# mahdeslami11/jalil-saboorizadeh-Multi-speaker-Neural-Vocoder

Hardware: AMD Instinct MI355X
Metric: audio samples/sec gen (3-tier dim1024) + TBPTT steps/sec @1/2/4/8 GPU (higher is better)
Workload: dtype bf16

## Files before the change

include/samplernn_hip.h:

```cpp
#ifndef SAMPLERNN_HIP_H
#define SAMPLERNN_HIP_H
#include <stddef.h>
#include <stdint.h>

#ifdef __cplusplus
extern "C" {
#endif

#define SRNN_MAX_TIERS 6
#define SRNN_MAX_RNN 4

const char* srnn_last_error(void);
int srnn_abi_version(void);
const char* srnn_build_hash(void);

int srnn_uquantize_f32(const float* x, int64_t* out, int64_t n, int q_levels, void* stream);
int srnn_uquantize_f64(const double* x, int64_t* out, int64_t n, int q_levels, void* stream);
int srnn_udequantize(const int64_t* k, float* out, int64_t n, int q_levels, float scale,
                     int mode, void* stream);
int srnn_udequantize2d(const int64_t* k, int64_t ldk, float* out, int rows, int cols,
                       int q_levels, float scale, int mode, void* stream);

int srnn_gemm(int dtype, int out_dtype, int transA, int transB, int M, int N, int K,
              float alpha, const void* A, int64_t lda, int64_t strideA, const void* B,
// ... 84 lines not shown
int srnn_gemm_amax_taken(void);
int srnn_gemm_amax_blk_next(unsigned* amax, void* blk);
int srnn_gemm_csum_next(float* part);
int srnn_gemm_csum_taken(void);
int srnn_gemm_logsoftmax_next(void);
int srnn_gemm_logsoftmax_taken(void);
int srnn_mlp_dtab4(int dtype, const void* da, int64_t ldda, const int64_t* x, int64_t ldx,
                   int xoff, int B, int Tlen, void* dtab_out, int out_dtype, int D, int FS0, int Q,
                   void* work, size_t work_bytes, float* colsum, int* colsum_done,
                   const unsigned* amax_in, const void* blk, void* stream);
int srnn_dtab_packed_ok(void);
int srnn_blaslt_calls(void);
int srnn_blaslt_set_min(long long min_outputs, double min_flop);
int srnn_blaslt_set_tune(int n);
int srnn_logsoftmax_bwd(const float* dlogp, int64_t lddl, const float* logp, int64_t ldl,
                        int64_t rows, int Q, void* dz, int dz_dtype, int64_t ldd, void* stream);
int srnn_nll_fwd(const float* logp, int64_t ldl, const int64_t* target, int64_t ldt, int Tlen,
                 int64_t rows, float* loss_row, void* stream);
int srnn_nll_bwd(const int64_t* target, int64_t ldt, int Tlen, int64_t rows, int Q,
                 float* dlogp, int64_t ldd, float gscale, const float* gmul, void* stream);
int srnn_nll_logsoftmax_bwd(const int64_t* target, int64_t ldt, int Tlen, int64_t rows, int Q,
                            const float* logp, int64_t ldl, float gscale, const float* gmul,
                            void* dz, int dz_dtype, int64_t ldd, void* stream);
int srnn_logsoftmax_nll(const float* z, int64_t ldz, const int64_t* target, int64_t ldt,
                        int Tlen, int64_t rows, int Q, float* loss_row, float* logp,
                        int64_t ldl, void* dz, int dz_dtype, int64_t ldd, float gscale,
                        void* stream);

int srnn_uquantize_f64_host(const double* x, int64_t* out, int64_t n, int q_levels);
int srnn_uquantize_f32_host(const float* x, int64_t* out, int64_t n, int q_levels);
int srnn_udequantize_host(const int64_t* k, float* out, int64_t n, int q_levels);

int srnn_weight_norm_fwd(const float* g, const float* v, float* w, float* norm, int O,
                         int64_t R, void* stream);
int srnn_weight_norm_bwd(const float* g, const float* v, const float* dw, float* dg, float* dv,
                         int O, int64_t R, int accumulate, void* stream);
int srnn_weight_norm_scale(const float* g, const float* v, float* scale, int O, int64_t R,
                           void* stream);
int srnn_convt_fold(const float* v, const float* scale, void* dst, int dst_dtype, int Cin,
                    int Cout, int k, void* stream);
int srnn_convt_wn_bwd(const float* g, const float* v, const float* dwt, float* dg, float* dv,
                      int Cin, int Cout, int k, void* stream);

int srnn_permute3(const float* src, void* dst, int dst_dtype, int d0, int d1, int d2, int p0,
                  int p1, int p2, int accumulate, void* stream);
int srnn_copy2d(int src_dtype, int dst_dtype, int rows, int cols, const void* src, int64_t lds,
                void* dst, int64_t ldd, void* stream);
int srnn_gather_rows(const float* table, int64_t ldt, const int64_t* idx, int64_t n, int cols,
                     void* out, int out_dtype, int64_t ldo, void* stream);
int srnn_scatter_add_rows(float* table, int64_t ldt, const int64_t* idx, int64_t n, int cols,
                          const float* src, int64_t lds, void* stream);
int srnn_index_add_rows(float* table, int64_t ldt, int trows, const int64_t* idx, int64_t n,
                        int cols, const float* src, int64_t lds, void* stream);
int srnn_axpby(float* out, const float* a, const float* b, float alpha, float beta, int64_t n,
               void* stream);
int srnn_add_bcast_rows(float* x, const float* v, int B, int F, int D, int64_t ldv, void* stream);
int srnn_segsum(const float* src, int64_t lds, int B, int F, int D, float* out, void* stream);
int srnn_colsum(int dtype, const void* src, int64_t lds, int64_t rows, int cols, float* out,
                float alpha, int accumulate, float* work, int64_t work_elems, void* stream);

int srnn_adam_clip(float* p, float* g, float* m, float* v, void* p_bf16, int64_t n,
                   float clip_lo, float clip_hi, double lr, double beta1, double beta2,
                   double eps, int64_t step, void* stream);
int srnn_adam_clip_multi(int ntensors, float* const* p, float* const* g, float* const* m,
                         float* const* v, void* const* p_bf16, const int64_t* n, float clip_lo,
                         float clip_hi, double lr, double beta1, double beta2, double eps,
                         int64_t step, void* stream);
int srnn_adam_clip_multi2(int ntensors, float* const* p, void* const* g, int gdtype, float gscale,
                          float* const* m, float* const* v, void* const* p_bf16, const int64_t* n,
                          float clip_lo, float clip_hi, double lr, double beta1, double beta2,
                          double eps, int64_t step, void* stream);
int srnn_adam_clip_multi3(int ntensors, float* const* p, void* const* g, int gdtype, float gscale,
                          float* const* m, float* const* v, void* const* p_bf16, const int64_t* n,
                          float clip_lo, float clip_hi, double lr, double beta1, double beta2,
                          double eps, int64_t step, const int64_t* dstep, void* stream);
int srnn_step_advance(int64_t* dstep, int n, void* stream);
int srnn_pack_grads(int ntensors, const float* const* src, const int64_t* n,
                    const int64_t* dst_off, void* flat, int dtype, void* stream);
int srnn_cast_multi(int ntensors, const float* const* src, void* const* dst, const int64_t* n,
                    void* stream);

typedef struct SrnnTier {
// ... 44 lines not shown
```

jalil-saboorizadeh-multi-speaker-neural-vocoder_amd/csrc/misc.hip:

```cpp
#include <type_traits>
#include <algorithm>

#include "samplernn_hip_internal.hpp"
#include "ulaw_tables.h"

__constant__ uint32_t c_ulaw_f32_steps[256];
__constant__ uint64_t c_ulaw_f64_thresh[256];
__constant__ uint32_t c_ulaw_lut[256];

static int g_tables_ready = 0;
static int ensure_tables() {
    if (g_tables_ready) return 0;
    SRNN_CHECK_HIP(hipMemcpyToSymbol(HIP_SYMBOL(c_ulaw_f32_steps), SRNN_ULAW_F32_STEPS_BITS,
                                     sizeof(SRNN_ULAW_F32_STEPS_BITS)));
    SRNN_CHECK_HIP(hipMemcpyToSymbol(HIP_SYMBOL(c_ulaw_f64_thresh), SRNN_ULAW_F64_THRESH_BITS,
                                     sizeof(SRNN_ULAW_F64_THRESH_BITS)));
    SRNN_CHECK_HIP(hipMemcpyToSymbol(HIP_SYMBOL(c_ulaw_lut), SRNN_ULAW_LUT_BITS,
                                     sizeof(SRNN_ULAW_LUT_BITS)));
    g_tables_ready = 1;
    return 0;
}
int srnn_init_tables() { return ensure_tables(); }

__device__ __forceinline__ int64_t uq_formula(double x, int q) {
// ... 707 lines not shown
    s = block_sum(s, sh);
    if (threadIdx.x == 0) dst[c] = accumulate ? dst[c] + alpha * s : alpha * s;
}

template <typename T>
static void colsum_pass(const T* src, int64_t lds, int64_t rows, int cols, int64_t rpb, int nrb,
                        float* dst, float alpha, int accumulate, bool final_, hipStream_t s) {
    const bool vec = (lds % 4 == 0) && ((uintptr_t)src % (4 * sizeof(T)) == 0);
    dim3 grid(cdiv(cols, 64), nrb);
    if (final_ && cols < 16 && nrb == 1) {
        hipLaunchKernelGGL((colsum_narrow_kernel<T>), dim3(cols), dim3(256), 0, s, src, lds, rows,
                           dst, alpha, accumulate);
        return;
    }
    if (final_) {
        if (vec) hipLaunchKernelGGL((colsum_kernel<T, true, true>), grid, dim3(256), 0, s, src, lds, rows, cols, rpb, dst, alpha, accumulate);
        else hipLaunchKernelGGL((colsum_kernel<T, false, true>), grid, dim3(256), 0, s, src, lds, rows, cols, rpb, dst, alpha, accumulate);
    } else {
        if (vec) hipLaunchKernelGGL((colsum_kernel<T, true, false>), grid, dim3(256), 0, s, src, lds, rows, cols, rpb, dst, alpha, accumulate);
        else hipLaunchKernelGGL((colsum_kernel<T, false, false>), grid, dim3(256), 0, s, src, lds, rows, cols, rpb, dst, alpha, accumulate);
    }
}

int srnn_colsum_impl(int dtype, const void* src, int64_t lds, int64_t rows, int cols, float* out,
                     float alpha, int accumulate, float* work, int64_t work_elems, hipStream_t s) {
    if (cols <= 0) return 0;
    const int cblk = cdiv(cols, 64);
    int64_t nrb = std::max<int64_t>(1, std::min<int64_t>(2048 / cblk, rows / 64));
    nrb = std::min<int64_t>(nrb, work_elems / cols);
    if (rows <= 256 && cblk >= 16) nrb = 1;
    if (rows <= 0 || nrb <= 1) {
        if (dtype == SRNN_F32)
            colsum_pass<float>((const float*)src, lds, rows, cols, std::max<int64_t>(rows, 1), 1,
                               out, alpha, accumulate, true, s);
        else
            colsum_pass<bf16>((const bf16*)src, lds, rows, cols, std::max<int64_t>(rows, 1), 1,
                              out, alpha, accumulate, true, s);
        SRNN_LAUNCH_CHECK();
        return 0;
    }
    const int64_t rpb = (rows + nrb - 1) / nrb;
    nrb = (rows + rpb - 1) / rpb;
    SRNN_REQUIRE(nrb * cols <= work_elems, "colsum: workspace too small");
    if (dtype == SRNN_F32)
        colsum_pass<float>((const float*)src, lds, rows, cols, rpb, (int)nrb, work, 1.f, 0, false, s);
    else
        colsum_pass<bf16>((const bf16*)src, lds, rows, cols, rpb, (int)nrb, work, 1.f, 0, false, s);
    SRNN_LAUNCH_CHECK();
    colsum_pass<float>(work, cols, nrb, cols, nrb, 1, out, alpha, accumulate, true, s);
    SRNN_LAUNCH_CHECK();
    return 0;
}

__global__ void segsum_kernel(const float* __restrict__ src, int64_t lds, int B, int F, int D,
                              float* __restrict__ out) {
    const int c = blockIdx.x * blockDim.x + threadIdx.x;
    const int b = blockIdx.y;
    if (c >= D) return;
    const float* p = src + (int64_t)b * F * lds + c;
    float s = 0.f;
    for (int f = 0; f < F; ++f) s += p[(int64_t)f * lds];
    out[(int64_t)b * D + c] = s;
}

extern "C" int srnn_segsum(const float* src, int64_t lds, int B, int F, int D, float* out,
                           void* stream) {
    if ((int64_t)B * D <= 0) return 0;
    hipLaunchKernelGGL(segsum_kernel, dim3(cdiv(D, 256), B), dim3(256), 0, (hipStream_t)stream,
                       src, lds, B, F, D, out);
    SRNN_LAUNCH_CHECK();
    return 0;
}

extern "C" int srnn_colsum(int dtype, const void* src, int64_t lds, int64_t rows, int cols,
                           float* out, float alpha, int accumulate, float* work,
                           int64_t work_elems, void* stream) {
    return srnn_colsum_impl(dtype, src, lds, rows, cols, out, alpha, accumulate, work, work_elems,
                            (hipStream_t)stream);
}

__global__ void adam_clip_kernel(float* __restrict__ p, float* __restrict__ g,
                                 float* __restrict__ m, float* __restrict__ v,
                                 bf16* __restrict__ p_lp, int64_t n, float lo, float hi, float w1,
                                 float b2, float omb2, float step_size, float bc2s, float eps) {
    int64_t i = (int64_t)blockIdx.x * blockDim.x + threadIdx.x;
    if (i >= n) return;
    float gi = fminf(fmaxf(g[i], lo), hi);
    g[i] = gi;
    float mi = m[i];
    mi = mi + w1 * (gi - mi);
    float vi = v[i] * b2;
    vi = vi + omb2 * gi * gi;
    float denom = sqrtf(vi) / bc2s + eps;
    float pi = p[i] + (-step_size) * mi / denom;
    m[i] = mi;
    v[i] = vi;
    p[i] = pi;
    if (p_lp) p_lp[i] = __float2bfloat16(pi);
}

#define ADAM_MT 64
// ... 288 lines not shown
```

jalil-saboorizadeh-multi-speaker-neural-vocoder_amd/csrc/mlp.hip:

```cpp
#include <algorithm>

#include "samplernn_hip_internal.hpp"
#include "sampler.hpp"

template <typename T, typename TU, int VPT>
__global__ __launch_bounds__(256) void mlp_l1_kernel(const T* __restrict__ tab,
                                                     const int64_t* __restrict__ x, int64_t ldx,
                                                     int xoff, const int* __restrict__ base,
                                                     int Tlen, const TU* __restrict__ upper,
                                                     int64_t ldu, T* __restrict__ out, int64_t ldo,
                                                     int D, int FS0, int Q) {
    const int64_t r = blockIdx.y;
    const int b = r / Tlen, t = r % Tlen;
    const int off = xoff + (base ? *base : 0);
    const int64_t* xr = x + (int64_t)b * ldx + off + t;
    const int o0 = (blockIdx.x * 256 + threadIdx.x) * VPT;
    if (o0 >= D) return;
    float acc[VPT];
    const TU* ur = upper + r * ldu + o0;
#pragma unroll
    for (int j = 0; j < VPT; ++j) acc[j] = to_f(ur[j]);
    constexpr int KMAX = 32;
    int qs[KMAX];
#pragma unroll
// ... 432 lines not shown
#pragma unroll
    for (int j = 0; j < 4; ++j) dz[r * ldd + lane + 64 * j] = from_f<TG>(g[j] - expf(p[j]) * s);
}

extern "C" int srnn_nll_logsoftmax_bwd(const int64_t* target, int64_t ldt, int Tlen,
                                       int64_t rows, int Q, const float* logp, int64_t ldl,
                                       float gscale, const float* gmul, void* dz, int dz_dtype,
                                       int64_t ldd, void* stream) {
    SRNN_REQUIRE(Q == 256, "nll_logsoftmax_bwd: q_levels must be 256");
    if (rows <= 0) return 0;
    dim3 grid(cdiv(rows, 4));
    if (dz_dtype == SRNN_BF16)
        hipLaunchKernelGGL((nll_logsoftmax_bwd_kernel<bf16>), grid, dim3(256), 0,
                           (hipStream_t)stream, target, ldt, Tlen, rows, logp, ldl, gscale, gmul,
                           (bf16*)dz, ldd);
    else
        hipLaunchKernelGGL((nll_logsoftmax_bwd_kernel<float>), grid, dim3(256), 0,
                           (hipStream_t)stream, target, ldt, Tlen, rows, logp, ldl, gscale, gmul,
                           (float*)dz, ldd);
    SRNN_LAUNCH_CHECK();
    return 0;
}

__global__ void nll_fwd_kernel(const float* __restrict__ lp, int64_t ldl,
                               const int64_t* __restrict__ target, int64_t ldt, int Tlen,
                               int64_t rows, float* __restrict__ loss_row) {
    const int64_t r = (int64_t)blockIdx.x * blockDim.x + threadIdx.x;
    if (r >= rows) return;
    const int64_t b = r / Tlen, t = r % Tlen;
    loss_row[r] = -lp[r * ldl + target[b * ldt + t]];
}

__global__ void nll_bwd_kernel(const int64_t* __restrict__ target, int64_t ldt, int Tlen,
                               int64_t rows, int Q, float* __restrict__ dl, int64_t ldd,
                               float gscale, const float* __restrict__ gmul) {
    const int64_t e = (int64_t)blockIdx.x * blockDim.x + threadIdx.x;
    if (e >= rows * Q) return;
    if (gmul) gscale *= *gmul;
    const int64_t r = e / Q;
    const int q = e % Q;
    const int64_t b = r / Tlen, t = r % Tlen;
    dl[r * ldd + q] = (q == target[b * ldt + t]) ? -gscale : 0.f;
}

extern "C" int srnn_nll_fwd(const float* logp, int64_t ldl, const int64_t* target, int64_t ldt,
                            int Tlen, int64_t rows, float* loss_row, void* stream) {
// ... 79 lines not shown
```

jalil-saboorizadeh-multi-speaker-neural-vocoder_amd/csrc/samplernn_hip_internal.hpp:

```cpp
#pragma once
#include "gemm_problem.hpp"

int srnn_relu_bits_impl(int dtype, const void* a, int64_t lda, int M, int N, unsigned short* bits,
                        int64_t ldb, hipStream_t s);

__host__ __device__ __forceinline__ int64_t srnn_bits_index(int64_t r, int g, int64_t M, int64_t ld) {
    return ld ? r * ld + g : (int64_t)g * M + r;
}

static inline int linear_fwd(int dt, int odt, int M, int N, int K, const void* x, int64_t ldx,
                             const void* W, int64_t ldw, const float* bias, void* y, int64_t ldy,
                             int relu, hipStream_t s, float beta = 0.f, const float* yin = nullptr,
                             int64_t ldyin = 0) {
    GemmProblem p;
    p.dtype = dt; p.out_dtype = odt; p.transB = 1;
    p.M = M; p.N = N; p.K = K; p.beta = beta;
    p.A = x; p.lda = ldx; p.B = W; p.ldb = ldw; p.C = y; p.ldc = ldy;
    p.Cin = yin; p.ldcin = ldyin; p.bias = bias; p.bias_mode = 1; p.relu = relu;
    return srnn_gemm_run(p, s);
}

int srnn_raise_lds(const void* kernel, int bytes);

static inline int env_flag(const char* name, int dflt) {
    const char* e = getenv(name);
    return (e && *e) ? atoi(e) : dflt;
}

int* srnn_sticky_flag();
int srnn_persist_spin_limit(int dflt);
int srnn_device_cus();
extern "C" int srnn_device_share(void);
int srnn_persist_fits_cus(int64_t blocks);
int srnn_persist_check(const void* kernel, int threads, size_t lds, int64_t blocks,
                       const char* what);

enum { SRNN_SCRATCH_SPLITK = 0, SRNN_SCRATCH_MASK = 1, SRNN_SCRATCH_NT = 2, SRNN_SCRATCH_BLASLT = 3,
       SRNN_SCRATCH_SLOTS = 4 };
void* srnn_scratch(int slot, size_t bytes);

float* srnn_splitk_scratch(size_t bytes);
int srnn_splitk_sum(const float* part, float* C, int64_t ldc, int M, int N, int ks, hipStream_t s);

int srnn_blaslt_enabled();
```

jalil-saboorizadeh-multi-speaker-neural-vocoder_amd/model.py:

```python
import ctypes
import os

import numpy as np
import torch
from torch.nn import init

import custom_ops
import nn
import utils
import samplernn_hip as H

verbose = False
_STATS = {'fused_colsum': 0, 'fused_lp': 0, 'csum_epi': 0, 'lsm_epi': 0, 'gru_xcd_fwd': 0, 'gru_xcd_bwd': 0, 'gru_seq': 0,
          'gru_cell_steps': 0, 'gru_cell_bwd_steps': 0}


def _default_dtype():
    v = os.environ.get('SRNN_COMPUTE_DTYPE', 'fp32').lower()
    return torch.bfloat16 if v in ('bf16', 'bfloat16') else torch.float32


class _GRUParams(torch.nn.Module):

    def __init__(self, input_size, hidden_size, num_layers):
        super().__init__()
        self.input_size, self.hidden_size, self.num_layers = input_size, hidden_size, num_layers
        for l in range(num_layers):
            isz = input_size if l == 0 else hidden_size
            self.register_parameter('weight_ih_l%d' % l,
                                    torch.nn.Parameter(torch.empty(3 * hidden_size, isz)))
            self.register_parameter('weight_hh_l%d' % l,
                                    torch.nn.Parameter(torch.empty(3 * hidden_size, hidden_size)))
            self.register_parameter('bias_ih_l%d' % l,
                                    torch.nn.Parameter(torch.empty(3 * hidden_size)))
            self.register_parameter('bias_hh_l%d' % l,
                                    torch.nn.Parameter(torch.empty(3 * hidden_size)))
        stdv = 1.0 / np.sqrt(hidden_size)
# ... 5 lines not shown

    def __init__(self, frame_sizes, n_rnn, dim, learn_h0, q_levels, ulaw, weight_norm, cond_dim,
                 spk_dim, qrnn=False):
        super().__init__()
        self.dim = dim
        self.q_levels = q_levels
        self.ulaw = ulaw
        self.cond_dim = cond_dim
        self.spk_dim = spk_dim
        self.frame_sizes = [int(f) for f in frame_sizes]
        self.n_rnn = n_rnn
        self.compute_dtype = _default_dtype()
        self.dequantize = utils.udequantize if ulaw else utils.linear_dequantize
        ns_frame_samples = list(map(int, np.cumprod(frame_sizes)))
        is_cond = [False] * len(frame_sizes)
        is_cond[-1] = True
        self.frame_level_rnns = torch.nn.ModuleList([
            FrameLevelRNN(frame_size, n_frame_samples, n_rnn, dim, learn_h0, c, cond_dim,
                          spk_dim, weight_norm, qrnn)
            for (frame_size, n_frame_samples, c) in zip(frame_sizes, ns_frame_samples, is_cond)
        ])
        self.sample_level_mlp = SampleLevelMLP(frame_sizes[0], dim, q_levels, weight_norm)
        self.frame_level_rnns[0].__dict__['_feeds_mlp'] = True
        for m in self.modules():
            if m is not self:
                m.__dict__['_root'] = self

    @property
    def lookback(self):
        return self.frame_level_rnns[-1].n_frame_samples


class FrameLevelRNN(torch.nn.Module):

    def __init__(self, frame_size, n_frame_samples, n_rnn, dim, learn_h0, is_cond, cond_dim,
                 spk_dim, w_norm, qrnn):
        super().__init__()
        self.frame_size = frame_size
        self.n_frame_samples = n_frame_samples
        self.dim = dim
        self.cond_dim = cond_dim
        self.spk_dim = spk_dim
        self.weight_norm = w_norm
        self.qrnn = qrnn
        self.n_rnn = n_rnn
        self.is_cond = is_cond
# ... 83 lines not shown
    if T is not None:
        return T
    root = mod.__dict__.get('_root')
    return root.compute_dtype if root is not None else torch.float32


class _Conv:

    def __init__(self, ts):
        if len(ts) == 2:
            self.weight_g, self.weight_v = ts
        else:
            self.weight = ts[0]


class TierSpec:

    def __init__(self, meta, ps):
        (self.dim, self.n_frame_samples, self.frame_size, self.n_rnn, is_cond, feeds, dt,
         wn_ie, wn_c, wn_s, wn_up) = [int(v) for v in meta[:11]]
        self.is_cond = bool(is_cond)
        self.T = torch.bfloat16 if dt else torch.float32
        self._feeds_mlp = bool(feeds)
        it = iter(ps)

        def take(wn):
            return _Conv([next(it) for _ in range(2 if wn else 1)])
        self.input_expand = take(wn_ie)
        next(it)
        if self.is_cond:
            self.cond_expand = take(wn_c)
            next(it)
            next(it)
            self.spk_expand = take(wn_s)
            next(it)
        for _ in range(4 * self.n_rnn):
            next(it)
        self.upsampling = _State()
        self.upsampling.conv_t = take(wn_up)


def tier_meta(mod):
    wn = lambda m: int(hasattr(m, 'weight_g'))
    return [mod.dim, mod.n_frame_samples, mod.frame_size, mod.n_rnn, int(mod.is_cond),
            int(bool(mod.__dict__.get('_feeds_mlp'))), H.dcode(_dt(mod)),
            wn(mod.input_expand), wn(mod.cond_expand) if mod.is_cond else 0,
            wn(mod.spk_expand) if mod.is_cond else 0, wn(mod.upsampling.conv_t)]


class MlpSpec:

    def __init__(self, meta, ps):
        self.q_levels, self.dim, self.frame_size, dt, wn = [int(v) for v in meta[:5]]
        self.T = torch.bfloat16 if dt else torch.float32
        it = iter(ps)

        def take():
            return _Conv([next(it) for _ in range(2 if wn else 1)])
        self.embedding = _Conv([next(it)])
        self.input = take()
        self.hidden = take()
        self.hidden.bias = next(it)
        self.output = take()
        self.output.bias = next(it)


def mlp_meta(mlp):
    return [mlp.q_levels, mlp.dim, mlp.frame_size, H.dcode(_dt(mlp)),
            int(hasattr(mlp.hidden, 'weight_g'))]

# ... 141 lines not shown
    r = sv[9:]
    Wih, Whh = r[:L], r[L:2 * L]
    xs, outs, outsT, gates = r[2 * L:3 * L], r[3 * L:4 * L], r[4 * L:5 * L], r[5 * L:6 * L]
    WhhF = r[6 * L:7 * L]
    hprevs = r[7 * L:8 * L]
    dev = dY.device
    st = H.stream
    M = B * Fr
    if dY.dtype == T:
        dY2 = dYT = dY.reshape(M, k * D).contiguous()
    else:
        dY2 = dY.reshape(M, k * D).float().contiguous()
        lpc = getattr(dY, '_srnn_lp', None)
        if lpc is not None and lpc[1] == dY._version and lpc[0].dtype == T and \
                lpc[0].numel() == dY2.numel() and dY2.data_ptr() == dY.data_ptr():
            dYT = lpc[0].reshape(M, k * D)
            _STATS['fused_lp'] += 1
        else:
            dYT = H.cast(dY2, T)
    dWupT = H.gemm(outsT[-1].reshape(M, D), dYT, transA=True)
    cs = getattr(dY, '_srnn_colsum', None)
    if cs is not None and cs[1] == dY._version and cs[2] == k and cs[0].numel() == k * D:
        db_up = cs[0]
        _STATS['fused_colsum'] += 1
    else:
        db_up = H.colsum(dY2, M, k * D)
    dX = H.gemm(dYT, W_up.reshape(k * D, D))
    g_up = nn.convt_grad_to_params(mod.upsampling.conv_t, dWupT)
    g_up_b = H.permute3(db_up.reshape(1, k, D), (0, 2, 1)).reshape(D, k)
    g_rnn = [None] * L
    dh_in = [None] * L
    for l in reversed(range(L)):
        dOut = dX.reshape(B, Fr, D)
        WhhT = H.permute3(WhhF[l].detach().reshape(1, 3 * D, D), (0, 2, 1), dtype=T)
        xbw = H.gru_xcd_bwd_work_bytes(T, B, D) if lp else 0
        seq = lp and (xbw > 0 or H.gru_seq_supported(T, B, D))
        ddir = [torch.empty((B, D), device=dev, dtype=torch.float32) for _ in range(2)]
        dGIT = bsum = None
        if xbw > 0:
            dGH = dGI = None
            dGHT = torch.empty((B, Fr, 3 * D), device=dev, dtype=T)
            dGIT = torch.empty((B, Fr, 3 * D), device=dev, dtype=T)
            bsum = torch.empty((B, 4 * D), device=dev, dtype=torch.float32)
        else:
            dGH = torch.empty((B, Fr, 3 * D), device=dev, dtype=torch.float32)
            dGHT = torch.empty((B, Fr, 3 * D), device=dev, dtype=T) if lp else dGH
            dGI = torch.empty((B, Fr, 3 * D), device=dev, dtype=torch.float32)
# ... 39 lines not shown
        hprevT = hprevs[l]
        if hprevT is None:
            hprevT = torch.empty((B, Fr, D), device=dev, dtype=T)
            H.lib().call('srnn_copy2d', H.F32, H.dcode(T), B, D, H.ptr(h_in[l]), D,
                         H.ptr(hprevT), Fr * D, st())
            if Fr > 1:
                H.lib().call('srnn_copy2d', H.dcode(T), H.dcode(T), B, (Fr - 1) * D,
                             H.ptr(outsT[l]), Fr * D, H.ptr(hprevT[:, 1:]), Fr * D, st())
        dW_hh = H.gemm(dGHT.reshape(M, 3 * D), hprevT.reshape(M, D), transA=True)
        if bsum is not None:
            bs = H.colsum(bsum, B, 4 * D)
            db_hh = bs[:3 * D]
            db_ih = torch.cat([bs[:2 * D], bs[3 * D:]])
            dGIT = dGIT.reshape(M, 3 * D)
        else:
            dGH2, dGI2 = dGH.reshape(M, 3 * D), dGI.reshape(M, 3 * D)
            db_hh = H.colsum(dGH2, M, 3 * D)
            dGIT = H.cast(dGI2, T)
            db_ih = H.colsum(dGI2, M, 3 * D)
        dW_ih = H.gemm(dGIT, xs[l], transA=True)
        dX = H.gemm(dGIT, Wih[l])
        g_rnn[l] = [dW_ih, dW_hh, db_ih, db_hh]
    dx0 = dX
    dx0T = H.cast(dx0, T)
    dW_ie = H.gemm(dx0T, prevT, transA=True)
    g_ie = nn.weight_grad_to_params(mod.input_expand, dW_ie.reshape(D, nfs, 1))
    g_ie_b = H.colsum(dx0, M, D)
    d_upper = dx0.reshape(B, Fr, D) if ctx.has_upper else None
    if d_upper is not None and dx0T is not dx0:
        d_upper._srnn_lp = (dx0T, d_upper._version)
    grads = g_ie + [g_ie_b]
    if mod.is_cond:
        C = condT.shape[1]
        S = spk_embT.shape[1]
        dW_c = H.gemm(dx0T, condT, transA=True)
        grads += nn.weight_grad_to_params(mod.cond_expand, dW_c.reshape(D, C, 1))
        grads += [g_ie_b.clone()]
        dspk = torch.empty((B, D), device=dev, dtype=torch.float32)
        H.lib().call('srnn_segsum', H.ptr(dx0), D, B, Fr, D, H.ptr(dspk), st())
        dspkT = H.cast(dspk, T)
        dW_s = H.gemm(dspkT, spk_embT, transA=True)
        db_s = H.colsum(dspk, B, D)
        demb = H.gemm(dspkT, W_s)
        dE = torch.zeros((S, S), device=dev, dtype=torch.float32)
        H.lib().call('srnn_index_add_rows', H.ptr(dE), S, S, H.ptr(spk_flat), B, S,
                     H.ptr(demb), S, st())
        grads += [dE]
        grads += nn.weight_grad_to_params(mod.spk_expand, dW_s.reshape(D, S, 1))
        grads += [db_s]
    for l in range(L):
        grads += g_rnn[l]
    grads += g_up + [g_up_b]
    dh0 = None
# ... 100 lines not shown
        logp = torch.empty((B * Tl, Q), device=dev, dtype=torch.float32)
        H.lib().call('srnn_logsoftmax_nll', H.ptr(z), Q, None, 0, Tl, B * Tl, Q, None,
                     H.ptr(logp), Q, None, H.F32, 0, 0.0, H.stream())
    ctx = _State()
    ctx.mlp = mlp
    ctx.T = T
    ctx.udt = upper.dtype
    ctx.dims = (B, Tl, D, Q, FS0)
    ctx.saved_tensors = (x, a1, a2, logp, Wp, ET, W_hid, W_out)
    ctx.bits = (m1, m2)
    ctx.W_t = W_t
    return logp.reshape(B, Tl, Q), ctx


def mlp_backward(ctx, dlogp, nll=None):
    mlp = ctx.mlp
    T = ctx.T
    B, Tl, D, Q, FS0 = ctx.dims
    x, a1, a2, logp, Wp, ET, W_hid, W_out = ctx.saved_tensors
    dev = logp.device
    st = H.stream
    M = B * Tl
    dz = torch.empty((M, Q), device=dev, dtype=T)
    if nll is not None:
        tg, Tt, gscale, gd = nll
        H.lib().call('srnn_nll_logsoftmax_bwd', H.ptr(tg), Tt, Tt, M, Q, H.ptr(logp), Q,
                     gscale, H.ptr(gd), H.ptr(dz), H.dcode(T), Q, st())
    else:
        dl = dlogp.reshape(M, Q).float().contiguous()
        H.lib().call('srnn_logsoftmax_bwd', H.ptr(dl), Q, H.ptr(logp), Q, M, Q, H.ptr(dz),
                     H.dcode(T), Q, st())
    dW_out = H.gemm(dz, a2, transA=True)
    db_out = H.colsum(dz, M, Q)
    m1, m2 = ctx.bits
    ctx.bits = None
    W_t = ctx.W_t
    ctx.W_t = None
    Wo, tB = (W_t[1], True) if W_t is not None else (W_out, False)
    csp = None
    if T == torch.bfloat16 and M % 256 == 0 and os.environ.get('SRNN_CSUM_EPI', '1') != '0':
        csp = torch.empty((M // 128, D), device=dev, dtype=torch.float32)
        H.lib().call('srnn_gemm_csum_next', H.ptr(csp))
    ev = H.roof_begin()
    if m2 is not None:
        da2 = H.gemm(dz, Wo, transB=tB, mask_bits=m2, out_dtype=T)
    else:
        da2 = H.gemm(dz, Wo, transB=tB, mask=a2, out_dtype=T)
    H.roof_end('mlp_da2_gemm', ev, 2.0 * M * D * Q)
    if csp is not None and not H.lib().dll.srnn_gemm_csum_taken():
        csp = None
    if csp is not None:
        _STATS['csum_epi'] += 1
    ev = H.roof_begin()
    dW_hid = H.gemm(da2, a1, transA=True)
    H.roof_end('mlp_dw_hid_gemm', ev, 2.0 * M * D * D)
    db_hid = H.colsum(csp, M // 128, D) if csp is not None else H.colsum(da2, M, D)
# ... 289 lines not shown
```

jalil-saboorizadeh-multi-speaker-neural-vocoder_amd/samplernn_hip.py:

```python
import ctypes
import sys
import time
import os
import weakref

import torch

HERE = os.path.dirname(os.path.abspath(__file__))
LIB_PATH = os.path.join(HERE, 'libsamplernn_hip.so')

F32, BF16 = 0, 1
MAX_TIERS, MAX_RNN = 6, 4

_P = ctypes.c_void_p
_I = ctypes.c_int
_L = ctypes.c_int64
_F = ctypes.c_float
_D = ctypes.c_double
_U64 = ctypes.c_uint64
_SZ = ctypes.c_size_t

_SIGS = {
    'srnn_uquantize_f32': [_P, _P, _L, _I, _P],
    'srnn_uquantize_f64': [_P, _P, _L, _I, _P],
# ... 54 lines not shown
    'srnn_gru_xcd_bwd': [_I, _I, _I, _I, _P, _L, _L, _P, _L, _L, _P, _L, _L, _P, _P, _P, _P, _P,
                         _L, _L, _P, _P, _SZ, _P],
    'srnn_gru_xcd_bwd2': [_I, _I, _I, _I, _P, _L, _L, _P, _L, _L, _P, _L, _L, _P, _P, _P, _P, _P,
                          _P, _P, _L, _L, _P, _P, _SZ, _P],
    'srnn_weight_norm_scale': [_P, _P, _P, _I, _L, _P],
    'srnn_convt_fold': [_P, _P, _P, _I, _I, _I, _I, _P],
    'srnn_convt_wn_bwd': [_P, _P, _P, _P, _P, _I, _I, _I, _P],
    'srnn_gen_workspace_size': [_P, _I, ctypes.POINTER(_SZ)],
    'srnn_generate': [_P, _I, _I, _P, _P, _P, _U64, _P, _P, _P, _SZ, _I, _P],
    'srnn_generate2': [_P, _I, _I, _P, _P, _P, _U64, _I, _P, _P, _P, _SZ, _I, _P],
    'srnn_generate3': [_P, _I, _I, _P, _P, _P, _U64, _I, _P, _P, _P, _SZ, _I, _P, _P, _P],
    'srnn_persistent_flag_to_f32': [_P, _P],
    'srnn_persistent_flag_or_f32': [_P, _P],
    'srnn_persistent_flag_snapshot': [_P, _P],
    'srnn_persistent_flag_to': [_P, _I, _P],
    'srnn_persistent_flag_or': [_P, _I, _P],
    'srnn_adam_clip_multi2': [_I, _P, _P, _I, _F, _P, _P, _P, _P, _F, _F, _D, _D, _D, _D, _L,
                              _P],
    'srnn_pack_grads': [_I, _P, _P, _P, _P, _I, _P],
    'srnn_adam_clip_multi3': [_I, _P, _P, _I, _F, _P, _P, _P, _P, _F, _F, _D, _D, _D, _D, _L,
                              _P, _P],
    'srnn_step_advance': [_P, _I, _P],
    'srnn_nll_logsoftmax_bwd': [_P, _L, _I, _L, _I, _P, _L, _F, _P, _P, _I, _L, _P],
}


class SrnnTier(ctypes.Structure):
    _fields_ = [('frame_size', _I), ('n_frame_samples', _I), ('in_dim', _I),
                ('w_in', _P), ('b_in', _P),
                ('w_ih', _P * MAX_RNN), ('b_ih', _P * MAX_RNN),
                ('w_hh', _P * MAX_RNN), ('b_hh', _P * MAX_RNN),
                ('w_up', _P), ('b_up', _P), ('h0', _P)]


class SrnnModel(ctypes.Structure):
    _fields_ = [('n_tiers', _I), ('n_rnn', _I), ('dim', _I), ('q_levels', _I),
                ('cond_dim', _I), ('dtype', _I), ('tier', SrnnTier * MAX_TIERS),
                ('tab', _P), ('w_hid', _P), ('b_hid', _P), ('w_out', _P), ('b_out', _P)]


class _Lib:
    def __init__(self, path):
        if not os.path.exists(path):
            raise ImportError('libsamplernn_hip.so not built (%s); run __graft_entry__.build()'
                              % path)
        self.dll = ctypes.CDLL(path)
# ... 336 lines not shown
    if out is None:
        out = torch.empty(cols, device=x.device, dtype=torch.float32)
    lds = cols if lds is None else lds
    nrb = max(1, min((rows + 63) // 64, 2048 // max(1, (cols + 63) // 64)))
    work = torch.empty(nrb * cols + 256, device=x.device, dtype=torch.float32)
    lib().call('srnn_colsum', dcode(x), ptr(x), lds, rows, cols, ptr(out), alpha, int(accumulate),
               ptr(work), work.numel(), stream())
    return out


def cast(x, dtype):
    need_cuda(x)
    if x.dtype == dtype:
        return x
    x = x.contiguous()
    out = torch.empty(x.shape, device=x.device, dtype=dtype)
    cols = x.shape[-1] if x.dim() > 0 else 1
    rows = x.numel() // max(cols, 1)
    lib().call('srnn_copy2d', dcode(x), dcode(out), rows, cols, ptr(x), cols, ptr(out), cols,
               stream())
    return out


_SHADOW = {}


def cast_param(p, dtype):
    if p.dtype == dtype:
        return p
    key = id(p)
    e = _SHADOW.get(key)
    if e is not None and e[0]() is p and e[1].dtype == dtype and e[2] == p.data_ptr() and \
            e[3] == p._version:
        return e[1]
    c = cast(p.detach(), dtype)
    if e is None or e[0]() is not p:
        weakref.finalize(p, _SHADOW.pop, key, None)
    _SHADOW[key] = (weakref.ref(p), c, p.data_ptr(), p._version)
    return c


def shadow_refreshed(p):
    e = _SHADOW.get(id(p))
    if e is not None and e[0]() is p and e[2] == p.data_ptr():
        _SHADOW[id(p)] = (e[0], e[1], p.data_ptr(), p._version)

# ... 67 lines not shown
```

Measured before the change: 40.71 million.

## Fuse column sums into NLL-logsoftmax backward and dx0 bf16 cast

Adds a kernel that computes the bf16 dz gradient of NLL+logsoftmax and accumulates its per-column bias gradient partials in the same pass. Also adds a fused cast+colsum kernel for the tier input gradient that emits the bf16 copy, the total column sum, and the k-strided sums the upper tier's upsampling bias gradient needs, so the upper tier can reuse them. The aim is to drop separate colsum passes over dz and dx0 in TBPTT backward. The dz column sum is now taken from the bf16-rounded values rather than a separate read.

```diff
diff --git a/include/samplernn_hip.h b/include/samplernn_hip.h
--- a/include/samplernn_hip.h
+++ b/include/samplernn_hip.h
@@ -130,6 +130,10 @@
 int srnn_nll_logsoftmax_bwd(const int64_t* target, int64_t ldt, int Tlen, int64_t rows, int Q,
                             const float* logp, int64_t ldl, float gscale, const float* gmul,
                             void* dz, int dz_dtype, int64_t ldd, void* stream);
+int srnn_nll_logsoftmax_bwd_csum(const int64_t* target, int64_t ldt, int Tlen, int64_t rows,
+                                 int Q, const float* logp, int64_t ldl, float gscale,
+                                 const float* gmul, void* dz, int dz_dtype, int64_t ldd,
+                                 float* part, int64_t part_rows, float* colsum, void* stream);
 int srnn_logsoftmax_nll(const float* z, int64_t ldz, const int64_t* target, int64_t ldt,
                         int Tlen, int64_t rows, int Q, float* loss_row, float* logp,
                         int64_t ldl, void* dz, int dz_dtype, int64_t ldd, float gscale,
@@ -166,6 +170,9 @@
 int srnn_segsum(const float* src, int64_t lds, int B, int F, int D, float* out, void* stream);
 int srnn_colsum(int dtype, const void* src, int64_t lds, int64_t rows, int cols, float* out,
                 float alpha, int accumulate, float* work, int64_t work_elems, void* stream);
+int srnn_cast_colsum(const float* src, int64_t lds, int64_t rows, int cols, int k, void* dst,
+                     int dst_dtype, int64_t ldd, float* sums, float* total, float* work,
+                     int64_t work_elems, void* stream);
 
 int srnn_adam_clip(float* p, float* g, float* m, float* v, void* p_bf16, int64_t n,
                    float clip_lo, float clip_hi, double lr, double beta1, double beta2,
diff --git a/jalil-saboorizadeh-multi-speaker-neural-vocoder_amd/csrc/misc.hip b/jalil-saboorizadeh-multi-speaker-neural-vocoder_amd/csrc/misc.hip
--- a/jalil-saboorizadeh-multi-speaker-neural-vocoder_amd/csrc/misc.hip
+++ b/jalil-saboorizadeh-multi-speaker-neural-vocoder_amd/csrc/misc.hip
@@ -753,13 +753,31 @@
     }
 }
 
-int srnn_colsum_impl(int dtype, const void* src, int64_t lds, int64_t rows, int cols, float* out,
-                     float alpha, int accumulate, float* work, int64_t work_elems, hipStream_t s) {
-    if (cols <= 0) return 0;
+int64_t srnn_colsum_plan(int64_t rows, int cols, int64_t work_elems, int64_t* rpb) {
     const int cblk = cdiv(cols, 64);
     int64_t nrb = std::max<int64_t>(1, std::min<int64_t>(2048 / cblk, rows / 64));
     nrb = std::min<int64_t>(nrb, work_elems / cols);
     if (rows <= 256 && cblk >= 16) nrb = 1;
+    if (rows <= 0 || nrb <= 1) {
+        *rpb = std::max<int64_t>(rows, 1);
+        return 1;
+    }
+    *rpb = (rows + nrb - 1) / nrb;
+    return (rows + *rpb - 1) / *rpb;
+}
+
+int srnn_colsum_final(const float* work, int64_t nrb, int cols, float* out, float alpha,
+                      int accumulate, hipStream_t s) {
+    colsum_pass<float>(work, cols, nrb, cols, nrb, 1, out, alpha, accumulate, true, s);
+    SRNN_LAUNCH_CHECK();
+    return 0;
+}
+
+int srnn_colsum_impl(int dtype, const void* src, int64_t lds, int64_t rows, int cols, float* out,
+                     float alpha, int accumulate, float* work, int64_t work_elems, hipStream_t s) {
+    if (cols <= 0) return 0;
+    int64_t rpb;
+    const int64_t nrb = srnn_colsum_plan(rows, cols, work_elems, &rpb);
     if (rows <= 0 || nrb <= 1) {
         if (dtype == SRNN_F32)
             colsum_pass<float>((const float*)src, lds, rows, cols, std::max<int64_t>(rows, 1), 1,
@@ -770,17 +788,13 @@
         SRNN_LAUNCH_CHECK();
         return 0;
     }
-    const int64_t rpb = (rows + nrb - 1) / nrb;
-    nrb = (rows + rpb - 1) / rpb;
     SRNN_REQUIRE(nrb * cols <= work_elems, "colsum: workspace too small");
     if (dtype == SRNN_F32)
         colsum_pass<float>((const float*)src, lds, rows, cols, rpb, (int)nrb, work, 1.f, 0, false, s);
     else
         colsum_pass<bf16>((const bf16*)src, lds, rows, cols, rpb, (int)nrb, work, 1.f, 0, false, s);
     SRNN_LAUNCH_CHECK();
-    colsum_pass<float>(work, cols, nrb, cols, nrb, 1, out, alpha, accumulate, true, s);
-    SRNN_LAUNCH_CHECK();
-    return 0;
+    return srnn_colsum_final(work, nrb, cols, out, alpha, accumulate, s);
 }
 
 __global__ void segsum_kernel(const float* __restrict__ src, int64_t lds, int B, int F, int D,
@@ -808,6 +822,132 @@
                            int64_t work_elems, void* stream) {
     return srnn_colsum_impl(dtype, src, lds, rows, cols, out, alpha, accumulate, work, work_elems,
                             (hipStream_t)stream);
+}
+
+__device__ __forceinline__ unsigned cc_pack2(float a, float b) {
+    const bf16 x = from_f<bf16>(a), y = from_f<bf16>(b);
+    return (unsigned)*reinterpret_cast<const unsigned short*>(&x) |
+           ((unsigned)*reinterpret_cast<const unsigned short*>(&y) << 16);
+}
+
+template <bool VEC>
+__global__ __launch_bounds__(256) void cast_colsum_kernel(const float* __restrict__ src,
+                                                          int64_t lds, bf16* __restrict__ dst,
+                                                          int64_t ldd, int64_t rows, int cols,
+                                                          int k, int64_t rpb,
+                                                          float* __restrict__ part) {
+    __shared__ float red[16][129];
+    const int tx = threadIdx.x & 15, ty = threadIdx.x >> 4;
+    const int c = blockIdx.x * 128 + tx * 8;
+    const int64_t r0 = (int64_t)blockIdx.y * rpb;
+    const int64_t r1 = min(rows, r0 + rpb);
+    float s[8];
+#pragma unroll
+    for (int e = 0; e < 8; ++e) s[e] = 0.f;
+    if (VEC && c + 7 < cols) {
+        int64_t r = r0 + ty;
+        for (; r + 16 < r1; r += 32) {
+            floatx4 v[2][2];
+#pragma unroll
+            for (int u = 0; u < 2; ++u) {
+                const floatx4* p = reinterpret_cast<const floatx4*>(src + (r + 16 * u) * lds + c);
+                v[u][0] = p[0]; v[u][1] = p[1];
+            }
+#pragma unroll
+            for (int u = 0; u < 2; ++u) {
+                uint4 o;
+                o.x = cc_pack2(v[u][0][0], v[u][0][1]); o.y = cc_pack2(v[u][0][2], v[u][0][3]);
+                o.z = cc_pack2(v[u][1][0], v[u][1][1]); o.w = cc_pack2(v[u][1][2], v[u][1][3]);
+                *reinterpret_cast<uint4*>(dst + (r + 16 * u) * ldd + c) = o;
+#pragma unroll
+                for (int e = 0; e < 4; ++e) { s[e] += v[u][0][e]; s[4 + e] += v[u][1][e]; }
+            }
+        }
+        for (; r < r1; r += 16) {
+            const floatx4* p = reinterpret_cast<const floatx4*>(src + r * lds + c);
+            const floatx4 v0 = p[0], v1 = p[1];
+            uint4 o;
+            o.x = cc_pack2(v0[0], v0[1]); o.y = cc_pack2(v0[2], v0[3]);
+            o.z = cc_pack2(v1[0], v1[1]); o.w = cc_pack2(v1[2], v1[3]);
+            *reinterpret_cast<uint4*>(dst + r * ldd + c) = o;
+#pragma unroll
+            for (int e = 0; e < 4; ++e) { s[e] += v0[e]; s[4 + e] += v1[e]; }
+        }
+    } else {
+        for (int64_t r = r0 + ty; r < r1; r += 16)
+#pragma unroll
+            for (int e = 0; e < 8; ++e)
+                if (c + e < cols) {
+                    const float v = src[r * lds + c + e];
+                    dst[r * ldd + c + e] = from_f<bf16>(v);
+                    s[e] += v;
+                }
+    }
+#pragma unroll
+    for (int e = 0; e < 8; ++e) red[ty][tx * 8 + e] = s[e];
+    __syncthreads();
+    for (int o = threadIdx.x; o < k * 128; o += 256) {
+        const int j = o >> 7, cc = o & 127;
+        float t = 0.f;
+        for (int i = j; i < 16; i += k) t += red[i][cc];
+        if (blockIdx.x * 128 + cc < cols)
+            part[((int64_t)blockIdx.y * k + j) * cols + blockIdx.x * 128 + cc] = t;
+    }
+}
+
+__global__ __launch_bounds__(256) void cc_final_kernel(const float* __restrict__ part, int nrb,
+                                                       int k, int cols, float* __restrict__ sums,
+                                                       float* __restrict__ total) {
+    __shared__ float red[16][17];
+    const int tx = threadIdx.x & 15, ty = threadIdx.x >> 4;
+    const int c = blockIdx.x * 16 + tx;
+    float tot = 0.f;
+    for (int j = 0; j < k; ++j) {
+        float s = 0.f;
+        if (c < cols)
+            for (int b = ty; b < nrb; b += 16) s += part[((int64_t)b * k + j) * cols + c];
+        red[ty][tx] = s;
+        __syncthreads();
+        if (ty == 0) {
+            float t = 0.f;
+#pragma unroll
+            for (int i = 0; i < 16; ++i) t += red[i][tx];
+            if (c < cols && sums) sums[(int64_t)j * cols + c] = t;
+            tot += t;
+        }
+        __syncthreads();
+    }
+    if (ty == 0 && c < cols) total[c] = tot;
+}
+
+extern "C" int srnn_cast_colsum(const float* src, int64_t lds, int64_t rows, int cols, int k,
+                                void* dst, int dst_dtype, int64_t ldd, float* sums,
+                                float* total, float* work, int64_t work_elems, void* stream) {
+    SRNN_REQUIRE(dst_dtype == SRNN_BF16, "cast_colsum: dst must be bf16");
+    SRNN_REQUIRE(k >= 1 && k <= 16 && 16 % k == 0, "cast_colsum: k must divide 16");
+    SRNN_REQUIRE(rows > 0 && cols > 0, "cast_colsum: empty input");
+    SRNN_REQUIRE(total != nullptr, "cast_colsum: total is required");
+    const int cblk = cdiv(cols, 128);
+    int64_t nrb = std::max<int64_t>(1, std::min<int64_t>(1024 / cblk, rows / 64));
+    int64_t rpb = (rows + nrb - 1) / nrb;
+    rpb = (rpb + 15) / 16 * 16;
+    nrb = (rows + rpb - 1) / rpb;
+    SRNN_REQUIRE(work && work_elems >= nrb * k * cols, "cast_colsum: workspace too small");
+    const bool vec = lds % 4 == 0 && ldd % 8 == 0 && (uintptr_t)src % 16 == 0 &&
+                     (uintptr_t)dst % 16 == 0;
+    hipStream_t s = (hipStream_t)stream;
+    dim3 grid(cblk, (unsigned)nrb);
+    if (vec)
+        hipLaunchKernelGGL((cast_colsum_kernel<true>), grid, dim3(256), 0, s, src, lds, (bf16*)dst,
+                           ldd, rows, cols, k, rpb, work);
+    else
+        hipLaunchKernelGGL((cast_colsum_kernel<false>), grid, dim3(256), 0, s, src, lds,
+                           (bf16*)dst, ldd, rows, cols, k, rpb, work);
+    SRNN_LAUNCH_CHECK();
+    hipLaunchKernelGGL(cc_final_kernel, dim3(cdiv(cols, 16)), dim3(256), 0, s, work, (int)nrb, k,
+                       cols, sums, total);
+    SRNN_LAUNCH_CHECK();
+    return 0;
 }
 
 __global__ void adam_clip_kernel(float* __restrict__ p, float* __restrict__ g,
diff --git a/jalil-saboorizadeh-multi-speaker-neural-vocoder_amd/csrc/mlp.hip b/jalil-saboorizadeh-multi-speaker-neural-vocoder_amd/csrc/mlp.hip
--- a/jalil-saboorizadeh-multi-speaker-neural-vocoder_amd/csrc/mlp.hip
+++ b/jalil-saboorizadeh-multi-speaker-neural-vocoder_amd/csrc/mlp.hip
@@ -478,6 +478,83 @@
     return 0;
 }
 
+__global__ __launch_bounds__(1024) void nll_logsoftmax_bwd_csum_kernel(
+    const int64_t* __restrict__ target, int64_t ldt, int Tlen, int64_t rows,
+    const float* __restrict__ lp, int64_t ldl, float gscale, const float* __restrict__ gmul,
+    bf16* __restrict__ dz, int64_t ldd, int64_t rpb, float* __restrict__ part) {
+    __shared__ float red[16][256];
+    const int wave = threadIdx.x >> 6, lane = threadIdx.x & 63;
+    if (gmul) gscale *= *gmul;
+    const int64_t r0 = (int64_t)blockIdx.x * rpb + wave;
+    const int64_t r1 = min(rows, (int64_t)(blockIdx.x + 1) * rpb);
+    float cs[4] = {0.f, 0.f, 0.f, 0.f};
+    int64_t b = r0 / Tlen;
+    int64_t t = r0 - b * Tlen;
+    for (int64_t rb = r0; rb < r1; rb += 64) {
+        int tq[4];
+        float p[4][4];
+#pragma unroll
+        for (int u = 0; u < 4; ++u) {
+            const int64_t r = rb + 16 * u;
+            if (r < r1) {
+                tq[u] = (int)target[b * ldt + t];
+#pragma unroll
+                for (int j = 0; j < 4; ++j) p[u][j] = lp[r * ldl + lane + 64 * j];
+                t += 16;
+                while (t >= Tlen) {
+                    t -= Tlen;
+                    ++b;
+                }
+            }
+        }
+#pragma unroll
+        for (int u = 0; u < 4; ++u) {
+            const int64_t r = rb + 16 * u;
+            if (r < r1) {
+                float g[4];
+#pragma unroll
+                for (int j = 0; j < 4; ++j) g[j] = (lane + 64 * j == tq[u]) ? -gscale : 0.f;
+                const float s = wave_sum(g[0] + g[1] + g[2] + g[3]);
+#pragma unroll
+                for (int j = 0; j < 4; ++j) {
+                    const bf16 v = from_f<bf16>(g[j] - expf(p[u][j]) * s);
+                    dz[r * ldd + lane + 64 * j] = v;
+                    cs[j] += to_f(v);
+                }
+            }
+        }
+    }
+#pragma unroll
+    for (int j = 0; j < 4; ++j) red[wave][lane + 64 * j] = cs[j];
+    __syncthreads();
+    if (threadIdx.x < 256) {
+        const int c = threadIdx.x;
+        float t = 0.f;
+#pragma unroll
+        for (int i = 0; i < 16; ++i) t += red[i][c];
+        part[(int64_t)blockIdx.x * 256 + c] = t;
+    }
+}
+
+extern "C" int srnn_nll_logsoftmax_bwd_csum(const int64_t* target, int64_t ldt, int Tlen,
+                                            int64_t rows, int Q, const float* logp, int64_t ldl,
+                                            float gscale, const float* gmul, void* dz,
+                                            int dz_dtype, int64_t ldd, float* part,
+                                            int64_t part_rows, float* colsum, void* stream) {
+    SRNN_REQUIRE(Q == 256, "nll_logsoftmax_bwd_csum: q_levels must be 256");
+    SRNN_REQUIRE(dz_dtype == SRNN_BF16, "nll_logsoftmax_bwd_csum: dz must be bf16");
+    SRNN_REQUIRE(colsum != nullptr, "nll_logsoftmax_bwd_csum: colsum is required");
+    if (rows <= 0) return 0;
+    int64_t rpb;
+    const int64_t nb = srnn_colsum_plan(rows, Q, INT64_MAX, &rpb);
+    SRNN_REQUIRE(part && part_rows >= nb, "nll_logsoftmax_bwd_csum: partials too small");
+    hipLaunchKernelGGL(nll_logsoftmax_bwd_csum_kernel, dim3((unsigned)nb), dim3(1024), 0,
+                       (hipStream_t)stream, target, ldt, Tlen, rows, logp, ldl, gscale, gmul,
+                       (bf16*)dz, ldd, rpb, part);
+    SRNN_LAUNCH_CHECK();
+    return srnn_colsum_final(part, nb, Q, colsum, 1.f, 0, (hipStream_t)stream);
+}
+
 __global__ void nll_fwd_kernel(const float* __restrict__ lp, int64_t ldl,
                                const int64_t* __restrict__ target, int64_t ldt, int Tlen,
                                int64_t rows, float* __restrict__ loss_row) {
diff --git a/jalil-saboorizadeh-multi-speaker-neural-vocoder_amd/csrc/samplernn_hip_internal.hpp b/jalil-saboorizadeh-multi-speaker-neural-vocoder_amd/csrc/samplernn_hip_internal.hpp
--- a/jalil-saboorizadeh-multi-speaker-neural-vocoder_amd/csrc/samplernn_hip_internal.hpp
+++ b/jalil-saboorizadeh-multi-speaker-neural-vocoder_amd/csrc/samplernn_hip_internal.hpp
@@ -42,4 +42,8 @@
 float* srnn_splitk_scratch(size_t bytes);
 int srnn_splitk_sum(const float* part, float* C, int64_t ldc, int M, int N, int ks, hipStream_t s);
 
+int64_t srnn_colsum_plan(int64_t rows, int cols, int64_t work_elems, int64_t* rpb);
+int srnn_colsum_final(const float* work, int64_t nrb, int cols, float* out, float alpha,
+                      int accumulate, hipStream_t s);
+
 int srnn_blaslt_enabled();
diff --git a/jalil-saboorizadeh-multi-speaker-neural-vocoder_amd/model.py b/jalil-saboorizadeh-multi-speaker-neural-vocoder_amd/model.py
--- a/jalil-saboorizadeh-multi-speaker-neural-vocoder_amd/model.py
+++ b/jalil-saboorizadeh-multi-speaker-neural-vocoder_amd/model.py
@@ -12,7 +12,8 @@
 
 verbose = False
 _STATS = {'fused_colsum': 0, 'fused_lp': 0, 'csum_epi': 0, 'lsm_epi': 0, 'gru_xcd_fwd': 0, 'gru_xcd_bwd': 0, 'gru_seq': 0,
-          'gru_cell_steps': 0, 'gru_cell_bwd_steps': 0}
+          'gru_cell_steps': 0, 'gru_cell_bwd_steps': 0, 'dz_csum': 0, 'dx0_fused': 0,
+          'tier_colsum': 0}
 
 
 def _default_dtype():
@@ -64,6 +65,8 @@
         ])
         self.sample_level_mlp = SampleLevelMLP(frame_sizes[0], dim, q_levels, weight_norm)
         self.frame_level_rnns[0].__dict__['_feeds_mlp'] = True
+        for lo, up in zip(self.frame_level_rnns[:-1], self.frame_level_rnns[1:]):
+            lo.__dict__['_upper_k'] = up.frame_size
         for m in self.modules():
             if m is not self:
                 m.__dict__['_root'] = self
@@ -193,6 +196,7 @@
         self.is_cond = bool(is_cond)
         self.T = torch.bfloat16 if dt else torch.float32
         self._feeds_mlp = bool(feeds)
+        self._upper_k = int(meta[11]) if len(meta) > 11 else 0
         it = iter(ps)
 
         def take(wn):
@@ -216,7 +220,8 @@
     return [mod.dim, mod.n_frame_samples, mod.frame_size, mod.n_rnn, int(mod.is_cond),
             int(bool(mod.__dict__.get('_feeds_mlp'))), H.dcode(_dt(mod)),
             wn(mod.input_expand), wn(mod.cond_expand) if mod.is_cond else 0,
-            wn(mod.spk_expand) if mod.is_cond else 0, wn(mod.upsampling.conv_t)]
+            wn(mod.spk_expand) if mod.is_cond else 0, wn(mod.upsampling.conv_t),
+            int(mod.__dict__.get('_upper_k') or 0)]
 
 
 class MlpSpec:
@@ -404,7 +409,7 @@
     cs = getattr(dY, '_srnn_colsum', None)
     if cs is not None and cs[1] == dY._version and cs[2] == k and cs[0].numel() == k * D:
         db_up = cs[0]
-        _STATS['fused_colsum'] += 1
+        _STATS[cs[3] if len(cs) > 3 else 'fused_colsum'] += 1
     else:
         db_up = H.colsum(dY2, M, k * D)
     dX = H.gemm(dYT, W_up.reshape(k * D, D))
@@ -490,13 +495,22 @@
         dX = H.gemm(dGIT, Wih[l])
         g_rnn[l] = [dW_ih, dW_hh, db_ih, db_hh]
     dx0 = dX
-    dx0T = H.cast(dx0, T)
+    k_up = int(getattr(mod, '_upper_k', 0) or 0) if ctx.has_upper else 1
+    cs_up = None
+    if T == torch.bfloat16 and dx0.dtype == torch.float32 and H.cast_colsum_ok(k_up) and \
+            M % k_up == 0 and os.environ.get('SRNN_DX0_FUSED', '1') != '0':
+        dx0T, cs_up, g_ie_b = H.cast_colsum(dx0, M, D, k_up)
+        _STATS['dx0_fused'] += 1
+    else:
+        dx0T = H.cast(dx0, T)
+        g_ie_b = H.colsum(dx0, M, D)
     dW_ie = H.gemm(dx0T, prevT, transA=True)
     g_ie = nn.weight_grad_to_params(mod.input_expand, dW_ie.reshape(D, nfs, 1))
-    g_ie_b = H.colsum(dx0, M, D)
     d_upper = dx0.reshape(B, Fr, D) if ctx.has_upper else None
     if d_upper is not None and dx0T is not dx0:
         d_upper._srnn_lp = (dx0T, d_upper._version)
+    if d_upper is not None and cs_up is not None:
+        d_upper._srnn_colsum = (cs_up.reshape(-1), d_upper._version, k_up, 'tier_colsum')
     grads = g_ie + [g_ie_b]
     if mod.is_cond:
         C = condT.shape[1]
@@ -643,16 +657,22 @@
     st = H.stream
     M = B * Tl
     dz = torch.empty((M, Q), device=dev, dtype=T)
+    db_out = None
     if nll is not None:
         tg, Tt, gscale, gd = nll
-        H.lib().call('srnn_nll_logsoftmax_bwd', H.ptr(tg), Tt, Tt, M, Q, H.ptr(logp), Q,
-                     gscale, H.ptr(gd), H.ptr(dz), H.dcode(T), Q, st())
+        if T == torch.bfloat16 and os.environ.get('SRNN_DZ_CSUM', '1') != '0':
+            db_out = H.nll_logsoftmax_bwd_csum(tg, Tt, M, Q, logp, gscale, gd, dz)
+            _STATS['dz_csum'] += 1
+        else:
+            H.lib().call('srnn_nll_logsoftmax_bwd', H.ptr(tg), Tt, Tt, M, Q, H.ptr(logp), Q,
+                         gscale, H.ptr(gd), H.ptr(dz), H.dcode(T), Q, st())
     else:
         dl = dlogp.reshape(M, Q).float().contiguous()
         H.lib().call('srnn_logsoftmax_bwd', H.ptr(dl), Q, H.ptr(logp), Q, M, Q, H.ptr(dz),
                      H.dcode(T), Q, st())
     dW_out = H.gemm(dz, a2, transA=True)
-    db_out = H.colsum(dz, M, Q)
+    if db_out is None:
+        db_out = H.colsum(dz, M, Q)
     m1, m2 = ctx.bits
     ctx.bits = None
     W_t = ctx.W_t
diff --git a/jalil-saboorizadeh-multi-speaker-neural-vocoder_amd/samplernn_hip.py b/jalil-saboorizadeh-multi-speaker-neural-vocoder_amd/samplernn_hip.py
--- a/jalil-saboorizadeh-multi-speaker-neural-vocoder_amd/samplernn_hip.py
+++ b/jalil-saboorizadeh-multi-speaker-neural-vocoder_amd/samplernn_hip.py
@@ -100,6 +100,9 @@
                               _P, _P],
     'srnn_step_advance': [_P, _I, _P],
     'srnn_nll_logsoftmax_bwd': [_P, _L, _I, _L, _I, _P, _L, _F, _P, _P, _I, _L, _P],
+    'srnn_nll_logsoftmax_bwd_csum': [_P, _L, _I, _L, _I, _P, _L, _F, _P, _P, _I, _L, _P, _L, _P,
+                                     _P],
+    'srnn_cast_colsum': [_P, _L, _L, _I, _I, _P, _I, _L, _P, _P, _P, _L, _P],
 }
 
 
@@ -482,6 +485,33 @@
     return out
 
 
+def nll_logsoftmax_bwd_csum(target, Tlen, rows, Q, logp, gscale, gmul, dz):
+    need_cuda(logp)
+    part = torch.empty((max(1, min(512, rows // 64)), Q), device=logp.device, dtype=torch.float32)
+    out = torch.empty(Q, device=logp.device, dtype=torch.float32)
+    lib().call('srnn_nll_logsoftmax_bwd_csum', ptr(target), Tlen, Tlen, rows, Q, ptr(logp), Q,
+               gscale, ptr(gmul), ptr(dz), BF16, Q, ptr(part), part.shape[0], ptr(out), stream())
+    return out
+
+
+def cast_colsum_ok(k):
+    return 1 <= k <= 16 and 16 % k == 0
+
+
+def cast_colsum(x, rows, cols, k=1):
+    need_cuda(x)
+    x = x.contiguous()
+    dev = x.device
+    out = torch.empty((rows, cols), device=dev, dtype=torch.bfloat16)
+    sums = torch.empty((k, cols), device=dev, dtype=torch.float32)
+    total = torch.empty(cols, device=dev, dtype=torch.float32)
+    nrb = max(1, min(1024 // ((cols + 127) // 128), rows // 64))
+    work = torch.empty(nrb * k * cols, device=dev, dtype=torch.float32)
+    lib().call('srnn_cast_colsum', ptr(x), cols, rows, cols, k, ptr(out), BF16, cols, ptr(sums),
+               ptr(total), ptr(work), work.numel(), stream())
+    return out, sums, total
+
+
 _SHADOW = {}
 
 
```

Result: no change. 41.07 million, median of 4 (+0.9%).
